# ethz-asl/ethzasl_brisk

Measured on AMD Instinct MI355X. Metric: frames/sec detect+describe @1080p (1/2/4/8 GPU); % HBM roofline, higher is better.
Workload: dtype u8

## Files before the change

ethzasl_brisk_amd/csrc/brisk_kernels.hip:

```cpp
#include <hip/hip_runtime.h>
#include <stdlib.h>

#include "brisk_common.h"
#include "brisk_device_detect.h"
#include "brisk_kernels.h"

#ifdef BRISK_HIP_TUNING
static int env_knob(const char* name, int dflt) {
  const char* v = getenv(name);
  return (v && *v) ? atoi(v) : dflt;
}
#else
#define env_knob(name, dflt) (dflt)
#endif


__device__ __forceinline__ BriskLayerView make_view(const BriskGeom& G, uint8_t* pyr, uint16_t* smap, int frame,
                                                    int l) {
  BriskLayerView v;
  const long base = (long)frame * G.pyr_elems + G.L[l].off;
  v.img = brisk_layer_img(G, pyr, frame, l);
  v.smap = smap + base;
  v.w = G.L[l].w;
  v.h = G.L[l].h;
// ... 940 lines not shown
      const int j = j0 + tid;
      const unsigned* t = tmp + ((long)l * n_in + j) * 8;
      const bool ok = j < cnt && t[7] != 0;
      const unsigned long long bal = __ballot(ok);
      if (lane == 0) wtot[wave] = __popcll(bal);
      __syncthreads();
      int wbase = 0, total = 0;
#pragma unroll
      for (int q = 0; q < 16; ++q) { wbase += (q < wave) ? wtot[q] : 0; total += wtot[q]; }
      const int pos = base + wbase + __popcll(bal & ((1ull << lane) - 1ull));
      if (ok && pos < kp_cap) {
        BriskKeyPoint kp;
        kp.x = __uint_as_float(t[0]); kp.y = __uint_as_float(t[1]); kp.size = __uint_as_float(t[2]); kp.angle = __uint_as_float(t[3]);
        kp.response = __uint_as_float(t[4]); kp.octave = (int)t[5]; kp.class_id = (int)t[6];
        kp_out[pos] = kp;
      }
      __syncthreads();
      if (tid == 0) base += total;
      __syncthreads();
    }
  }
  if (tid == 0) {
    counters[0].nkp = min(base, kp_cap);
    if (base > kp_cap) atomicOr(&counters[0].overflow, 4);
  }
}

__global__ void __launch_bounds__(64) k_compute_scale(BriskGeom G, uint8_t* pyr, uint16_t* smap, const BriskKeyPoint* in, int n_in,
                                                       int suppress, BriskFrameCounters* counters, unsigned* det_scratch,
                                                       int det_cap, BriskKeyPoint* kp_out, int kp_cap, int always) {
  if (threadIdx.x != 0 || blockIdx.x != 0) return;
  if (!always && !counters[0].pad[0]) return;
  counters[0].full_clear = 1;
  BriskOrderedOut out;
  out.kp = kp_out; out.cap = kp_cap; out.n = 0; out.mask = nullptr; out.mask_row_pitch = 0;
  bool cap_exceeded = false;
  const bool undefined = brisk_compute_scale_walk(G, pyr, smap, in, n_in, suppress != 0, det_scratch, det_cap, &out, &cap_exceeded);
  if (undefined) atomicOr(&counters[0].overflow, 16);
  if (cap_exceeded) atomicOr(&counters[0].overflow, 1);
  counters[0].nkp = min(out.n, kp_cap);
  if (out.n > kp_cap) atomicOr(&counters[0].overflow, 4);
}

#ifndef TR_WAVES
#define TR_WAVES 16
#endif
#define TR_THREADS (TR_WAVES * 64)
#define TR_WIN 9
#ifndef TR_CHUNK
#define TR_CHUNK 3072
#endif
#define TR_PROG_DONE 0x7FFFFFFF
#define TR_DONE_BIT 4
#define TR_BM_WORDS 512
#ifdef TR_TIMING
#define TR_T(i) { const long long now_ = (long long)wall_clock64(); tacc[i] += (int)(now_ - tlast); tlast = now_; }
#else
#define TR_T(i)
#endif
#ifdef TR_TIMELINE
#define TR_STAMP(c_, l_, k_) if (c_) counters[frame].tl[(l_) * 8 + (k_)] = (int)wall_clock64();
#else
#define TR_STAMP(c_, l_, k_)
#endif


#define TR_KERNEL_NAME k_tie_resolve
#define TR_SORT_NAME tie_sort_large
#define TR_KERNEL_MASKS 0
#define TR_KERNEL_PAIR 0
#include "brisk_tie_kernel.inc"
#undef TR_KERNEL_NAME
#undef TR_KERNEL_MASKS
#undef TR_SORT_NAME
#define TR_KERNEL_NAME k_tie_resolve_small
#define TR_SORT_NAME tie_sort_large_small
#define TR_KERNEL_MASKS 1
#include "brisk_tie_kernel.inc"
#undef TR_KERNEL_NAME
#undef TR_SORT_NAME
#undef TR_KERNEL_PAIR
#define TR_KERNEL_NAME k_tie_resolve_pair
#define TR_SORT_NAME tie_sort_large_pair
#define TR_KERNEL_PAIR 1
#include "brisk_tie_kernel.inc"
#undef TR_KERNEL_NAME
#undef TR_KERNEL_PAIR
#undef TR_KERNEL_MASKS

#ifndef FN_THREADS
#define FN_THREADS 512
#endif
#define FN_BUCKETS 2048
#define FN_SMALL 3072
#define FN_SB 1024
__global__ void __launch_bounds__(FN_THREADS) k_finalize(BriskGeom G, const BriskCand* cand, BriskFrameCounters* counters,
                                                          unsigned* keys_scratch, BriskKeyPoint* kp_out, int cand_cap,
                                                          int kp_cap, const uint8_t* mask, long mask_pitch_frame,
                                                          int mask_row_pitch) {
  __shared__ int nvalid;
  __shared__ unsigned skey[FN_SMALL];
  __shared__ unsigned sidx[FN_SMALL];
  BRISK_CHAIN_SETPRIO();
  const int frame = blockIdx.x, tid = threadIdx.x;
  if (counters[frame].low_score) return;
  const int n = min(counters[frame].ncand, cand_cap);
  const BriskCand* C = cand + (long)frame * cand_cap;
  unsigned* keys = keys_scratch + (long)frame * cand_cap * 2;
  if (tid == 0) nvalid = 0;
  __syncthreads();
  constexpr int FN_U = 4;
  for (int i0 = tid; i0 < n; i0 += FN_U * FN_THREADS) {
    unsigned sw[FN_U], ck[FN_U];
#pragma unroll
    for (int u = 0; u < FN_U; ++u) {
      const int i = min(i0 + u * FN_THREADS, n - 1);
      sw[u] = *reinterpret_cast<const unsigned*>(reinterpret_cast<const uint8_t*>(&C[i]) + 4);
      ck[u] = C[i].key;
    }
#pragma unroll
    for (int u = 0; u < FN_U; ++u) {
      const int i = i0 + u * FN_THREADS;
      bool valid = i < n && ((sw[u] >> 16) & 0xFFu) == BRISK_ST_PASS && ((sw[u] >> 24) & 1u);
      if (valid && mask) {
        const BriskCand& c = C[i];
        const uint8_t* m = mask + (long)frame * mask_pitch_frame;
        valid = m[(long)(int)(c.ky + 0.5f) * mask_row_pitch + (int)(c.kx + 0.5f)] != 0;
      }
      if (valid) {
        const int j = atomicAdd(&nvalid, 1);
        keys[2 * j] = ck[u];
        keys[2 * j + 1] = (unsigned)i;
        if (j < FN_SMALL) { skey[j] = ck[u]; sidx[j] = (unsigned)i; }
      }
    }
  }
  __threadfence_block();
  __syncthreads();
  const int nv = nvalid;
  if (nv > FN_SMALL) {
    if (tid == 0) counters[frame].nvalid_large = nv;
    return;
  }
  {
    __shared__ int rbase[BRISK_MAX_LAYERS + 1];
    __shared__ int bhead[FN_SB];
    __shared__ int bstart[FN_SB];
    __shared__ int bnext[FN_SMALL];
    __shared__ int wsum[FN_THREADS / 64];
    if (tid == 0) {
      int acc = 0;
      for (int l = 0; l < G.nlayers; ++l) { rbase[l] = acc; acc += G.L[l].h; }
      rbase[G.nlayers] = acc;
    }
    for (int b = tid; b < FN_SB; b += FN_THREADS) { bhead[b] = -1; bstart[b] = 0; }
    __syncthreads();
    int shift = 0;
    while ((rbase[G.nlayers] >> shift) >= FN_SB) ++shift;
    auto bucket_of = [&](unsigned key) { return (rbase[key >> 26] + (int)((key >> 13) & 0x1FFF)) >> shift; };
    for (int j = tid; j < nv; j += FN_THREADS) {
      const int b = bucket_of(skey[j]);
      atomicAdd(&bstart[b], 1);
      bnext[j] = atomicExch(&bhead[b], j);
    }
    __syncthreads();
    {
      constexpr int PER = FN_SB / FN_THREADS;
      int loc[PER], sum = 0;
#pragma unroll
      for (int q = 0; q < PER; ++q) { loc[q] = bstart[tid * PER + q]; sum += loc[q]; }
      const int incl = wave_inclusive_scan(sum);
      const int lane = tid & 63, wave = tid >> 6;
      if (lane == 63) wsum[wave] = incl;
      __syncthreads();
      int woff = 0;
#pragma unroll
      for (int q = 0; q < FN_THREADS / 64; ++q) woff += (q < wave) ? wsum[q] : 0;
      int run = woff + incl - sum;
#pragma unroll
      for (int q = 0; q < PER; ++q) { bstart[tid * PER + q] = run; run += loc[q]; }
    }
    __syncthreads();
    for (int j = tid; j < nv; j += FN_THREADS) {
      const unsigned k = skey[j];
      const BriskCand& c = C[sidx[j]];
      const float4 r = *reinterpret_cast<const float4*>(&c.kx);
      const int lyr = c.layer;
      const int b = bucket_of(k);
      int rank = bstart[b];
      for (int q = bhead[b]; q >= 0; q = bnext[q]) rank += (skey[q] < k) ? 1 : 0;
      if (rank < kp_cap) {
        BriskKeyPoint kp;
        kp.x = r.x; kp.y = r.y; kp.size = r.z; kp.angle = -1.0f; kp.response = r.w;
        kp.octave = G.single_layer ? 0 : lyr; kp.class_id = -1;
        kp_out[(long)frame * kp_cap + rank] = kp;
      }
    }
  }
  if (tid == 0) {
    counters[frame].nkp = min(nv, kp_cap);
    if (nv > kp_cap) atomicOr(&counters[frame].overflow, 4);
  }
}

__global__ void __launch_bounds__(FN_THREADS) k_finalize_large(BriskGeom G, const BriskCand* cand, BriskFrameCounters* counters,
                                                                const unsigned* keys_scratch, unsigned* scratch2,
                                                                long scratch2_stride, BriskKeyPoint* kp_out, int cand_cap,
                                                                int kp_cap) {
  const int frame = blockIdx.x, tid = threadIdx.x;
  const int nv = counters[frame].nvalid_large;
  if (nv <= 0) return;
  __shared__ int bstart[FN_BUCKETS + 1];
  __shared__ int bfill[FN_BUCKETS];
  __shared__ int rbase[BRISK_MAX_LAYERS + 1];
  __shared__ int wsum[FN_THREADS / 64];
  const BriskCand* C = cand + (long)frame * cand_cap;
  const unsigned* keys = keys_scratch + (long)frame * cand_cap * 2;
  unsigned* tmp = scratch2 + (long)frame * scratch2_stride;
  if (tid == 0) {
    int acc = 0;
    for (int l = 0; l < G.nlayers; ++l) { rbase[l] = acc; acc += G.L[l].h; }
    rbase[G.nlayers] = acc;
  }
  for (int b = tid; b < FN_BUCKETS; b += FN_THREADS) { bstart[b] = 0; bfill[b] = 0; }
  __syncthreads();
  int shift = 0;
  while ((rbase[G.nlayers] >> shift) >= FN_BUCKETS) ++shift;
  for (int j = tid; j < nv; j += FN_THREADS) {
    const unsigned key = keys[2 * j];
    atomicAdd(&bstart[(rbase[key >> 26] + (int)((key >> 13) & 0x1FFF)) >> shift], 1);
  }
  __syncthreads();
  {
    constexpr int PER = FN_BUCKETS / FN_THREADS;
    int loc[PER], sum = 0;
#pragma unroll
    for (int q = 0; q < PER; ++q) { loc[q] = bstart[tid * PER + q]; sum += loc[q]; }
    int incl = sum;
    const int lane = tid & 63, wave = tid >> 6;
#pragma unroll
    for (int off = 1; off < 64; off <<= 1) {
      const int v = __shfl_up(incl, off, 64);
      if (lane >= off) incl += v;
    }
    if (lane == 63) wsum[wave] = incl;
    __syncthreads();
    int woff = 0;
#pragma unroll
    for (int q = 0; q < FN_THREADS / 64; ++q) woff += (q < wave) ? wsum[q] : 0;
    int run = woff + incl - sum;
#pragma unroll
    for (int q = 0; q < PER; ++q) { bstart[tid * PER + q] = run; run += loc[q]; }
    if (tid == FN_THREADS - 1) bstart[FN_BUCKETS] = run;
  }
  __syncthreads();
  for (int j = tid; j < nv; j += FN_THREADS) {
    const unsigned key = keys[2 * j];
    const int b = (rbase[key >> 26] + (int)((key >> 13) & 0x1FFF)) >> shift;
    const int pos = bstart[b] + atomicAdd(&bfill[b], 1);
    tmp[2 * pos] = key;
    tmp[2 * pos + 1] = keys[2 * j + 1];
  }
  __threadfence();
  __syncthreads();
  for (int pos = tid; pos < nv; pos += FN_THREADS) {
    const unsigned key = tmp[2 * pos];
    const int b = (rbase[key >> 26] + (int)((key >> 13) & 0x1FFF)) >> shift;
    int rank = bstart[b];
    for (int q = bstart[b]; q < bstart[b + 1]; ++q) rank += (tmp[2 * q] < key) ? 1 : 0;
    if (rank < kp_cap) {
      const BriskCand& c = C[tmp[2 * pos + 1]];
      BriskKeyPoint kp;
      kp.x = c.kx; kp.y = c.ky; kp.size = c.ksize; kp.angle = -1.0f; kp.response = c.kresp;
      kp.octave = G.single_layer ? 0 : c.layer; kp.class_id = -1;
      kp_out[(long)frame * kp_cap + rank] = kp;
    }
  }
  if (tid == 0) {
    counters[frame].nkp = min(nv, kp_cap);
    if (nv > kp_cap) atomicOr(&counters[frame].overflow, 4);
  }
}

#define II_THREADS 512
#define II_BAND 64
#define II_CHUNK (II_THREADS * 4)

__device__ __forceinline__ unsigned ii_wg_scan(unsigned total, unsigned (*wave_tot)[II_THREADS / 64], int buf, unsigned* wg_total) {
  const int lane = threadIdx.x & 63, wave = threadIdx.x >> 6;
  const unsigned incl = (unsigned)wave_inclusive_scan((int)total);
  if (lane == 63) wave_tot[buf][wave] = incl;
  __syncthreads();
  unsigned woff = 0, tot = 0;
#pragma unroll
  for (int q = 0; q < II_THREADS / 64; ++q) {
    const unsigned v = wave_tot[buf][q];
    woff += (q < wave) ? v : 0;
    tot += v;
  }
  *wg_total = tot;
  return woff + incl - total;
}

#ifndef II_ROWS
#define II_ROWS 3
#endif
#define II_MAXCHUNKS 4
__device__ __forceinline__ uint2 ii_fetch(const uint8_t* row, int stride, int c0 ) {
  const int a = min(max(c0 - 4, 0), stride - 4), b = min(c0, stride - 4);
  return make_uint2(*reinterpret_cast<const unsigned*>(row + a), *reinterpret_cast<const unsigned*>(row + b));
}
__device__ __forceinline__ void ii_unpack(uint2 raw, int stride, int w, int c0, unsigned* px) {
  const unsigned prev = (c0 >= 4 && c0 - 4 < stride) ? raw.x : 0u, cur = (c0 < stride) ? raw.y : 0u;
  px[0] = (c0 - 1 >= 0 && c0 - 1 < w) ? (prev >> 24) : 0;
  px[1] = (c0 < w) ? (cur & 0xFF) : 0;
  px[2] = (c0 + 1 < w) ? ((cur >> 8) & 0xFF) : 0;
  px[3] = (c0 + 2 < w) ? ((cur >> 16) & 0xFF) : 0;
}

typedef uint32_t __attribute__((ext_vector_type(3))) ii_u32x3;
__device__ __forceinline__ void ii_store4(bool b24, uint32_t* out, long row, int istride, int c0, unsigned a0, unsigned a1, unsigned a2, unsigned a3) {
  if (b24) {
    ii_u32x3 v;
    v.x = (a0 & 0xFFFFFFu) | (a1 << 24);
    v.y = ((a1 >> 8) & 0xFFFFu) | (a2 << 16);
    v.z = ((a2 >> 16) & 0xFFu) | (a3 << 8);
    *reinterpret_cast<ii_u32x3*>(reinterpret_cast<uint8_t*>(out) + (row * istride + c0) * 3) = v;
  } else {
    *reinterpret_cast<uint4*>(out + row * istride + c0) = make_uint4(a0, a1, a2, a3);
  }
}
template <int NCH, bool B24, bool SUB>
__global__ void __launch_bounds__(II_THREADS) k_integral_final(BriskGeom G, const uint8_t* __restrict__ pyr,
                                                               const uint32_t* __restrict__ bandsum,
                                                               uint32_t* __restrict__ integral, int istride, long iframe_elems,
                                                               int nbands, int band_h, BriskFrameCounters* counters, int nsub, int sub_h) {
  __shared__ unsigned wave_tot[2][II_THREADS / 64];
  const int frame = blockIdx.y, band = SUB ? (int)blockIdx.x / nsub : (int)blockIdx.x;
  const int sub = SUB ? (int)blockIdx.x - band * nsub : 0;
  constexpr bool b24 = B24;
  if (counters && blockIdx.x == 0 && threadIdx.x == 0) counters[frame].i24 = b24 ? 1 : 0;
  const int w = G.L[0].w, h = G.L[0].h, stride = G.L[0].stride;
  const uint8_t* img = brisk_layer_img(G, pyr, frame, 0);
  uint32_t* out = integral + (long)frame * iframe_elems;
  const int yb = band * band_h;
  const int y0 = SUB ? yb + sub * sub_h : yb;
  const int y1 = SUB ? min(min(h, yb + band_h), y0 + sub_h) : min(h, y0 + band_h);
  if (SUB && y0 >= y1) return;
  int buf = 0;
  unsigned acc[NCH][4];
  uint2 raw[NCH];
#pragma unroll
  for (int ch = 0; ch < NCH; ++ch) raw[ch] = ii_fetch(img + (long)min(y0, h - 1) * stride, stride, ch * II_CHUNK + threadIdx.x * 4);
  {
    unsigned carry = 0;
#pragma unroll
    for (int ch = 0; ch < NCH; ++ch) {
      const int c0 = ch * II_CHUNK + threadIdx.x * 4;
      uint4 C = make_uint4(0, 0, 0, 0);
      if (c0 <= w)
        for (int b = 0; b < band; ++b) {
          const uint4 v = *reinterpret_cast<const uint4*>(bandsum + ((long)frame * nbands + b) * istride + c0);
          C.x += v.x; C.y += v.y; C.z += v.z; C.w += v.w;
        }
      if (SUB && c0 <= w) {
        for (int r0 = yb; r0 < y0; r0 += 6) {
          uint2 rr[6];
#pragma unroll
          for (int k = 0; k < 6; ++k) rr[k] = ii_fetch(img + (long)min(r0 + k, y0 - 1) * stride, stride, c0);
#pragma unroll
          for (int k = 0; k < 6; ++k) {
            unsigned px[4];
            ii_unpack(rr[k], stride, w, c0, px);
            if (r0 + k < y0) { C.x += px[0]; C.y += px[1]; C.z += px[2]; C.w += px[3]; }
          }
        }
      }
      if (c0 + 1 > w) C.y = 0;
      if (c0 + 2 > w) C.z = 0;
      if (c0 + 3 > w) C.w = 0;
      const unsigned s0 = C.x, s1 = s0 + C.y, s2 = s1 + C.z, s3 = s2 + C.w;
      unsigned tot;
      const unsigned o = ii_wg_scan(s3, wave_tot, buf, &tot) + carry;
      buf ^= 1;
      carry += tot;
      acc[ch][0] = o + s0; acc[ch][1] = o + s1; acc[ch][2] = o + s2; acc[ch][3] = o + s3;
      if (band == 0 && sub == 0 && c0 <= w) ii_store4(b24, out, 0, istride, c0, 0, 0, 0, 0);
    }
  }
  __shared__ unsigned wave_totr[2][II_THREADS / 64][II_ROWS];
  uint2 rawr[II_ROWS][NCH];
#pragma unroll
  for (int k = 0; k < II_ROWS; ++k)
#pragma unroll
    for (int ch = 0; ch < NCH; ++ch)
      rawr[k][ch] = (k == 0) ? raw[ch] : ii_fetch(img + (long)min(y0 + k, h - 1) * stride, stride, ch * II_CHUNK + threadIdx.x * 4);
  const int lane = threadIdx.x & 63, wave = threadIdx.x >> 6;
  for (int y = y0; y < y1; y += II_ROWS) {
    uint2 nxt[II_ROWS][NCH];
#pragma unroll
    for (int k = 0; k < II_ROWS; ++k) {
      const int yn = min(y + II_ROWS + k, y1 - 1);
#pragma unroll
      for (int ch = 0; ch < NCH; ++ch) nxt[k][ch] = ii_fetch(img + (long)yn * stride, stride, ch * II_CHUNK + threadIdx.x * 4);
    }
    unsigned carry[II_ROWS];
#pragma unroll
    for (int k = 0; k < II_ROWS; ++k) carry[k] = 0;
#pragma unroll
    for (int ch = 0; ch < NCH; ++ch) {
      const int c0 = ch * II_CHUNK + threadIdx.x * 4;
      unsigned s[II_ROWS][4], incl[II_ROWS];
#pragma unroll
      for (int k = 0; k < II_ROWS; ++k) {
        unsigned px[4] = {0, 0, 0, 0};
        if (c0 <= w && y + k < y1) ii_unpack(rawr[k][ch], stride, w, c0, px);
        s[k][0] = px[0]; s[k][1] = s[k][0] + px[1]; s[k][2] = s[k][1] + px[2]; s[k][3] = s[k][2] + px[3];
        incl[k] = (unsigned)wave_inclusive_scan((int)s[k][3]);
        if (lane == 63) wave_totr[buf][wave][k] = incl[k];
      }
      __syncthreads();
#pragma unroll
      for (int k = 0; k < II_ROWS; ++k) {
        unsigned wo = 0, tot = 0;
#pragma unroll
        for (int q = 0; q < II_THREADS / 64; ++q) {
          const unsigned v = wave_totr[buf][q][k];
          wo += (q < wave) ? v : 0;
          tot += v;
        }
        const unsigned o = wo + incl[k] - s[k][3] + carry[k];
        carry[k] += tot;
        acc[ch][0] += o + s[k][0]; acc[ch][1] += o + s[k][1]; acc[ch][2] += o + s[k][2]; acc[ch][3] += o + s[k][3];
        if (c0 <= w && y + k < y1) ii_store4(b24, out, (long)(y + k + 1), istride, c0, acc[ch][0], acc[ch][1], acc[ch][2], acc[ch][3]);
      }
      buf ^= 1;
    }
#pragma unroll
    for (int k = 0; k < II_ROWS; ++k)
#pragma unroll
      for (int ch = 0; ch < NCH; ++ch) rawr[k][ch] = nxt[k][ch];
  }
}

void brisk_launch_integral(const BriskGeom& G, const uint8_t* pyr, const uint32_t* bandsum, uint32_t* integral, int istride,
                            long iframe_elems, int band_h, int nframes, hipStream_t s, int ibits, BriskFrameCounters* counters) {
  const int nbands = (G.L[0].h + band_h - 1) / band_h;
  const int nchunks = (G.L[0].w + 1 + II_CHUNK - 1) / II_CHUNK;
  static const int sub_knob = env_knob("BRISK_II_SUB", -1);
  const int sub_h = ((sub_knob > 0 ? sub_knob : (band_h >= 96 ? 18 : 15)) + II_ROWS - 1) / II_ROWS * II_ROWS;
  const bool sub = sub_knob != 0 && nframes <= 4 && sub_h < band_h;
  const int nsub = sub ? (band_h + sub_h - 1) / sub_h : 1;
  const dim3 grid(nbands * nsub, nframes), block(II_THREADS);
  static const int pad_lds = env_knob("BRISK_II_LDS", 0);
  const bool b24 = ibits == 24 && counters;
#define II_LAUNCH1(NCH, LDS, B24_, SUB_)                                                                                                   \
  hipLaunchKernelGGL((k_integral_final<NCH, B24_, SUB_>), grid, block, LDS, s, G, pyr, bandsum, integral, istride, iframe_elems, nbands,   \
                     band_h, counters, nsub, sub_h);
#define II_LAUNCH(NCH, LDS)                                                                                                                  \
  if (b24) { if (sub) { II_LAUNCH1(NCH, LDS, true, true) } else { II_LAUNCH1(NCH, LDS, true, false) } }                                      \
  else { if (sub) { II_LAUNCH1(NCH, LDS, false, true) } else { II_LAUNCH1(NCH, LDS, false, false) } }
  if (nchunks <= 1) { II_LAUNCH(1, pad_lds) }
  else if (nchunks == 2) { II_LAUNCH(2, 0) }
  else { II_LAUNCH(II_MAXCHUNKS, 0) }
#undef II_LAUNCH
#undef II_LAUNCH1
}

__global__ void __launch_bounds__(256) k_batch_density(const BriskFrameCounters* __restrict__ counters, int nframes, int cand_cap,
                                                       long long* __restrict__ host_word) {
  __shared__ long long part[4];
  long long sum = 0;
  for (int f = threadIdx.x; f < nframes; f += 256) sum += min(counters[f].ncand, cand_cap);
  for (int off = 32; off > 0; off >>= 1) sum += __shfl_xor(sum, off, 64);
  if ((threadIdx.x & 63) == 0) part[threadIdx.x >> 6] = sum;
  __syncthreads();
  if (threadIdx.x == 0) {
    const long long total = part[0] + part[1] + part[2] + part[3];
    __hip_atomic_store(host_word, (total & 0xFFFFFFFFFFll) | ((long long)nframes << 40), __ATOMIC_RELAXED, __HIP_MEMORY_SCOPE_SYSTEM);
  }
}
void brisk_launch_batch_density(const BriskFrameCounters* counters, int nframes, int cand_cap, long long* host_word, hipStream_t s) {
  hipLaunchKernelGGL(k_batch_density, dim3(1), dim3(256), 0, s, counters, nframes, cand_cap, host_word);
}

__global__ void __launch_bounds__(256) k_publish_single(const BriskFrameCounters* __restrict__ counters, const BriskKeyPoint* __restrict__ kps,
                                                        const uint8_t* __restrict__ desc, int which, int max_kp, int dev_pitch,
                                                        uint8_t* host, unsigned o_cnt, unsigned o_kp, unsigned o_desc, int* done, unsigned seq) {
  const int tid = threadIdx.x, gt = blockIdx.x * blockDim.x + tid, gn = gridDim.x * blockDim.x;
  const int cnt = (counters[0].overflow & 7) ? 0 : (which ? counters[0].ndesc : counters[0].nkp);
  const bool fits = cnt <= max_kp;
  const int n = fits ? cnt : 0;
  if (blockIdx.x == 0)
    for (int i = tid; i < (int)(sizeof(BriskFrameCounters) / 4); i += blockDim.x)
      reinterpret_cast<int*>(host + o_cnt)[i] = reinterpret_cast<const int*>(counters)[i];
  {
    const int* src = reinterpret_cast<const int*>(kps);
    int* dst = reinterpret_cast<int*>(host + o_kp);
    const int nd = n * (int)(sizeof(BriskKeyPoint) / 4);
    for (int i = gt; i < nd; i += gn) dst[i] = src[i];
  }
  if (desc) {
    const uint2* src = reinterpret_cast<const uint2*>(desc);
    uint2* dst = reinterpret_cast<uint2*>(host + o_desc);
    const long nd = (long)n * dev_pitch / 8;
    for (long i = gt; i < nd; i += gn) dst[i] = src[i];
  }
  __threadfence_system();
  __syncthreads();
  if (tid == 0) {
    const int old = __hip_atomic_fetch_add(done, 1, __ATOMIC_ACQ_REL, __HIP_MEMORY_SCOPE_AGENT);
    if (old == (int)gridDim.x - 1) {
      __hip_atomic_store(done, 0, __ATOMIC_RELAXED, __HIP_MEMORY_SCOPE_AGENT);
      __threadfence_system();
      __hip_atomic_store(reinterpret_cast<unsigned*>(host), seq | (fits ? 0u : 0x80000000u), __ATOMIC_RELEASE, __HIP_MEMORY_SCOPE_SYSTEM);
    }
  }
}
void brisk_launch_publish_single(const BriskFrameCounters* counters, const BriskKeyPoint* kps, const uint8_t* desc, int which, int max_kp,
                                 int dev_pitch, int expect, uint8_t* host, unsigned o_cnt, unsigned o_kp, unsigned o_desc, int* done,
                                 unsigned seq, hipStream_t s) {
  const long bytes = (long)expect * ((long)sizeof(BriskKeyPoint) + (desc ? dev_pitch : 0));
  int grid = (int)((bytes + 16383) / 16384);
  grid = grid < 1 ? 1 : (grid > 32 ? 32 : grid);
  hipLaunchKernelGGL(k_publish_single, dim3(grid), dim3(256), 0, s, counters, kps, desc, which, max_kp, dev_pitch, host, o_cnt, o_kp, o_desc,
                     done, seq);
}

int brisk_device_cus() {
  static int cus[64] = {};
  int dev = 0;
  if (hipGetDevice(&dev) != hipSuccess || dev < 0 || dev >= 64) return 256;
  int v = __atomic_load_n(&cus[dev], __ATOMIC_RELAXED);
  if (!v) {
    hipDeviceProp_t prop;
    v = (hipGetDeviceProperties(&prop, dev) == hipSuccess && prop.multiProcessorCount > 0) ? prop.multiProcessorCount : 256;
    __atomic_store_n(&cus[dev], v, __ATOMIC_RELAXED);
  }
  return v;
}

static inline int grid_for(long items, int per_block, int cap) {
  long b = (items + per_block - 1) / per_block;
  if (b < 1) b = 1;
  if (b > cap) b = cap;
  return (int)b;
}

const char* brisk_stage_name(int i) {
  static const char* n[BRISK_PROF_STAGES] = {"k_pyramid", "k_detect", "k_classify_refine", "k_tie_resolve", "k_finalize",
                                             "k_postfilter", "k_integral_final", "k_desc_prepare", "k_describe"};
  return (i >= 0 && i < BRISK_PROF_STAGES) ? n[i] : "?";
}

void brisk_prof_begin_call(BriskProfiler* P) {
  if (!P || !P->on) return;
  if (!P->created) {
    for (int c = 0; c < BRISK_PROF_MAX_CALLS; ++c)
      for (int k = 0; k <= BRISK_PROF_STAGES; ++k) (void)hipEventCreate(&P->ev[c][k]);
    for (int c = 0; c < BRISK_PROF_MAX_CALLS; ++c)
      for (int k = 0; k < 2; ++k) (void)hipEventCreate(&P->side_ev[c][k]);
    P->created = true;
  }
  const int c = P->calls % BRISK_PROF_MAX_CALLS;
  for (int k = 0; k <= BRISK_PROF_STAGES; ++k) P->used[c][k] = false;
  P->side_used[c] = false;
}

void brisk_prof_mark_side(BriskProfiler* P, int which, hipStream_t side) {
  if (!P || !P->on) return;
  const int c = P->calls % BRISK_PROF_MAX_CALLS;
  (void)hipEventRecord(P->side_ev[c][which], side);
  if (which == 1) P->side_used[c] = true;
}

void brisk_prof_destroy(BriskProfiler* P) {
  if (!P || !P->created) return;
  for (int c = 0; c < BRISK_PROF_MAX_CALLS; ++c) {
    for (int k = 0; k <= BRISK_PROF_STAGES; ++k) (void)hipEventDestroy(P->ev[c][k]);
    for (int k = 0; k < 2; ++k) (void)hipEventDestroy(P->side_ev[c][k]);
  }
  P->created = false;
}

void brisk_prof_mark(BriskProfiler* P, int slot, hipStream_t s) {
  if (!P || !P->on) return;
  const int c = P->calls % BRISK_PROF_MAX_CALLS;
  (void)hipEventRecord(P->ev[c][slot], s);
  P->used[c][slot] = true;
}

__global__ void __launch_bounds__(256) k_stream_copy(const float4* __restrict__ in, float4* __restrict__ out, long n) {
  for (long i = (long)blockIdx.x * blockDim.x + threadIdx.x; i < n; i += (long)gridDim.x * blockDim.x) out[i] = in[i];
}
__global__ void __launch_bounds__(256) k_stream_read(const float4* __restrict__ in, float* __restrict__ out, long n) {
  float s = 0;
  for (long i = (long)blockIdx.x * blockDim.x + threadIdx.x; i < n; i += (long)gridDim.x * blockDim.x) {
    const float4 v = in[i];
    s += v.x + v.y + v.z + v.w;
  }
  if (s == 1.2345f) out[0] = s;
}
void brisk_launch_stream_probe(const void* a, void* b, size_t bytes, int mode, hipStream_t s) {
  const long n = (long)(bytes / 16);
  if (mode == 0) hipLaunchKernelGGL(k_stream_copy, dim3(4096), dim3(256), 0, s, (const float4*)a, (float4*)b, n);
  else hipLaunchKernelGGL(k_stream_read, dim3(4096), dim3(256), 0, s, (const float4*)a, (float*)b, n);
}

void brisk_launch_smap_clear(const BriskGeom& Gprev, const BriskDetectBuffers& B, int nframes, hipStream_t s) {
  if (nframes > 0) hipLaunchKernelGGL(k_smap_clear, dim3(16, nframes), dim3(256), 0, s, Gprev, B.smap, B.cand, B.counters, B.cand_cap);
}

static void launch_pyramid(const BriskGeom& G, const BriskDetectBuffers& B, int nframes, const uint8_t* frames, long frame_pitch,
                           int row_pitch, hipStream_t s) {
  {
    const int even_levels = G.nlayers >= 7 ? 3 : G.nlayers >= 5 ? 2 : G.nlayers >= 3 ? 1 : 0;
    const int odd_levels = G.nlayers >= 8 ? 3 : G.nlayers >= 6 ? 2 : G.nlayers >= 4 ? 1 : G.nlayers >= 2 ? 0 : -1;
    const int ftx = (G.L[0].stride + 95) / 96, fty = (G.L[0].h + PF_BAND - 1) / PF_BAND;
    hipLaunchKernelGGL(k_pyramid_fused, dim3(ftx * fty, nframes), dim3(256), 0, s, G, frames, frame_pitch, row_pitch, B.pyr,
                       even_levels, odd_levels, ftx, fty, B.bandsum, B.istride);
    for (int l = 8; l < G.nlayers; ++l) {
      const long items = (long)(G.L[l].stride / 4) * G.L[l].h;
      hipLaunchKernelGGL(k_pyramid_level, dim3(grid_for(items, 256, 2048), nframes), dim3(256), 0, s, G, B.pyr, l - 2, l, 0);
    }
  }
}

void brisk_launch_detect(const BriskGeom& G, const BriskTileTable& T, const BriskDetectBuffers& B, int nframes,
                         const uint8_t* frames, long frame_pitch, int row_pitch, const uint8_t* mask,
                         long mask_frame_pitch, int mask_row_pitch, hipStream_t s, BriskProfiler* prof,
                         const BriskOverlap* ov) {
  (void)hipMemsetAsync(B.counters, 0, sizeof(BriskFrameCounters) * (size_t)nframes, s);
  brisk_prof_mark(prof, BRISK_STG_PYRAMID, s);
  const int probe_stop = env_knob("BRISK_DETECT_PROBE", 0);
  if (probe_stop != 2) launch_pyramid(G, B, nframes, frames, frame_pitch, row_pitch, s);
  static const int fork_at = env_knob("BRISK_INTEGRAL_FORK", 0);
  auto fork_integral = [&]() {
    (void)hipEventRecord(ov->fork, s);
    (void)hipStreamWaitEvent(ov->side, ov->fork, 0);
    brisk_prof_mark_side(prof, 0, ov->side);
    brisk_launch_integral(G, B.pyr, B.bandsum, ov->Dd->integral, ov->Dd->istride, ov->Dd->iframe_elems, B.band_h, nframes, ov->side,
                          ov->Dd->ibits, B.counters);
    brisk_prof_mark_side(prof, 1, ov->side);
    (void)hipEventRecord(ov->join, ov->side);
  };
  if (ov && fork_at == 1) fork_integral();
  brisk_prof_mark(prof, BRISK_STG_DETECT, s);
  hipLaunchKernelGGL(k_detect, dim3((T.total_tiles + 7) / 8 * 8, nframes), dim3(256), 0, s, G, T, B.pyr, B.smap, B.cand, B.counters,
                     B.cand_cap);
  if (probe_stop) return;
  if (ov && fork_at == 2) fork_integral();
  brisk_prof_mark(prof, BRISK_STG_CLASSIFY, s);
  const bool ordered_all = G.no_scale_nms || G.lower_threshold != BRISK_LOWER_THRESHOLD;
  const bool ordered_some = !ordered_all && G.threshold < BRISK_FAST_PATH_MIN_THRESHOLD;
  auto launch_ordered = [&](int only_flagged) {
    const long row_stride = (long)BRISK_MAX_LAYERS * B.tie_cap;
    hipLaunchKernelGGL(k_order_candidates, dim3(nframes), dim3(OC_THREADS), 0, s, G, B.cand, B.counters, B.keys, B.tie_idx,
                       row_stride, B.cand_cap, only_flagged);
    hipLaunchKernelGGL(k_ordered_keypoints, dim3(nframes), dim3(64), 0, s, G, B.pyr, B.smap, B.cand, B.counters, B.keys, B.kp_out,
                       B.cand_cap, B.kp_cap, mask, mask_frame_pitch, mask_row_pitch, G.no_scale_nms, only_flagged);
  };
  if (ordered_all) {
    brisk_prof_mark(prof, BRISK_STG_TIES, s);
    if (ov && fork_at != 1 && fork_at != 2) fork_integral();
    launch_ordered(0);
    brisk_prof_mark(prof, BRISK_STG_FINALIZE, s);
    brisk_prof_mark(prof, BRISK_STG_POSTFILTER, s);
    return;
  }
  static const int sb_knob = env_knob("BRISK_SB_BLOCKS", 0), cr_knob = env_knob("BRISK_CR_BLOCKS", 0);
  const int sb_blocks = sb_knob ? sb_knob : (nframes > 64 ? (nframes >= 256 ? 32 : 64) : 256), cr_blocks = cr_knob ? cr_knob : (nframes >= 64 ? 24 : 64);
  {
    const int sb_bpf = grid_for(B.cand_cap, SB_WAVES * SB_PER_WAVE, sb_blocks), cr_bpf = grid_for(B.cand_cap, 64, cr_blocks);
    hipLaunchKernelGGL(k_score_blocks, dim3(xcd_grid(nframes, sb_bpf)), dim3(SB_WAVES * 64), 0, s, G, B.pyr, B.smap, B.cand,
                       B.counters, B.blocks, B.cand_cap, nframes, sb_bpf);
    hipLaunchKernelGGL(k_classify_refine, dim3(xcd_grid(nframes, cr_bpf)), dim3(64), 0, s, G, B.pyr, B.smap, B.cand, B.counters,
                       B.blocks, B.tie_idx, B.cand_cap, B.tie_cap, nframes, cr_bpf);
  }
  hipLaunchKernelGGL(k_classify_refine_direct, dim3(8, nframes), dim3(64), 0, s, G, B.pyr, B.smap, B.cand, B.counters,
                     B.tie_idx, B.cand_cap, B.tie_cap);
  brisk_prof_mark(prof, BRISK_STG_TIES, s);
  if (ov && fork_at == 0) fork_integral();
  {
    static const int lpw_knob = env_knob("BRISK_TR_LPW", 0);
    const int per_wg = G.nlayers > 8 ? 192 : 256;
    int lpw_auto = G.nlayers;
    for (int c = 1; c <= G.nlayers; ++c)
      if (nframes * ((G.nlayers + c - 1) / c) <= per_wg) { lpw_auto = c; break; }
    const int lpw = lpw_knob ? min(lpw_knob, G.nlayers) : (nframes * G.nlayers <= 512 ? 1 : lpw_auto);
    int tr_grid = (nframes >= 8 ? (nframes + 7) / 8 * 8 : nframes) * ((G.nlayers + lpw - 1) / lpw);
    static const int persist_knob = env_knob("BRISK_TR_PERSIST", -1), pgrid_env = env_knob("BRISK_TR_PGRID", 0);
    const int pgrid_knob = pgrid_env > 0 ? pgrid_env : brisk_device_cus();
    const int persist = persist_knob >= 0 ? persist_knob : (tr_grid > pgrid_knob ? 1 : 0);
    if (persist && tr_grid > pgrid_knob) tr_grid = pgrid_knob;
    static const int waves_knob = env_knob("BRISK_TR_WAVES", 0);
    const int tr_waves = waves_knob ? min(max(waves_knob, 2), TR_WAVES) : ((!persist && lpw >= G.nlayers && nframes >= 192) ? 12 : TR_WAVES);
    static const int pair_knob = env_knob("BRISK_TR_PAIR", 1);
    static const int pair_min_knob = env_knob("BRISK_TR_PAIR_MIN", 0);
    static const int pair_mode_knob = env_knob("BRISK_TR_PAIR_MODE", 1);
    const int pair_min = (pair_min_knob ? pair_min_knob : 4 * (tr_waves - 1)) | (pair_mode_knob << 16);
    static const int bands_knob = env_knob("BRISK_TR_BANDS", 0);
    int bands = 1;
    if (lpw == 1 && !persist) {
      bands = bands_knob ? min(max(bands_knob, 1), BRISK_TIE_MAX_BANDS) : (tr_grid * 8 <= pgrid_knob ? 8 : tr_grid * 4 <= pgrid_knob ? 4 : tr_grid * 2 <= pgrid_knob ? 2 : 1);
      if (tr_grid * bands > pgrid_knob) bands = 1;
    }
    if ((nframes <= 64 && pair_knob) || pair_knob == 2)
      hipLaunchKernelGGL(k_tie_resolve_pair, dim3(tr_grid * bands), dim3(tr_waves * 64), 0, s, G, B.pyr, B.smap, B.cand, B.counters, B.tie_idx,
                         B.blocks, B.keys, B.cand_cap, B.tie_cap, nframes, lpw, persist, pair_min, bands);
    else if (nframes < 32)
      hipLaunchKernelGGL(k_tie_resolve_small, dim3(tr_grid), dim3(tr_waves * 64), 0, s, G, B.pyr, B.smap, B.cand, B.counters, B.tie_idx,
                         B.blocks, B.keys, B.cand_cap, B.tie_cap, nframes, lpw, persist, 0, 1);
    else
      hipLaunchKernelGGL(k_tie_resolve, dim3(tr_grid), dim3(tr_waves * 64), 0, s, G, B.pyr, B.smap, B.cand, B.counters, B.tie_idx,
                         B.blocks, B.keys, B.cand_cap, B.tie_cap, nframes, lpw, persist, 0, 1);
  }
  brisk_prof_mark(prof, BRISK_STG_FINALIZE, s);
  hipLaunchKernelGGL(k_finalize, dim3(nframes), dim3(FN_THREADS), 0, s, G, B.cand, B.counters, B.keys, B.kp_out, B.cand_cap,
                     B.kp_cap, mask, mask_frame_pitch, mask_row_pitch);
  hipLaunchKernelGGL(k_finalize_large, dim3(nframes), dim3(FN_THREADS), 0, s, G, B.cand, B.counters, B.keys,
                     reinterpret_cast<unsigned*>(B.tie_idx), (long)BRISK_MAX_LAYERS * B.tie_cap, B.kp_out, B.cand_cap, B.kp_cap);
  if (ordered_some) launch_ordered(1);
  brisk_prof_mark(prof, BRISK_STG_POSTFILTER, s);
}

void brisk_launch_compute_scale(const BriskGeom& G, const BriskDetectBuffers& B, const uint8_t* frame, int row_pitch,
                                const BriskKeyPoint* d_in, int n_in, int suppress, hipStream_t s) {
  (void)hipMemsetAsync(B.counters, 0, sizeof(BriskFrameCounters), s);
  launch_pyramid(G, B, 1, frame, 0, row_pitch, s);
  static const int seq_knob = env_knob("BRISK_CS_SEQUENTIAL", 0);
  const bool parallel = !seq_knob && (long)G.nlayers * n_in <= 2L * B.cand_cap;
  if (parallel) {
    int* adm = reinterpret_cast<int*>(B.keys);
    unsigned* tmp = reinterpret_cast<unsigned*>(B.blocks);
    hipLaunchKernelGGL(k_cs_admit, dim3(G.nlayers), dim3(CS_THREADS), 0, s, G, B.pyr, B.smap, d_in, n_in, B.counters, adm);
    hipLaunchKernelGGL(k_cs_scores, dim3((n_in + CS_THREADS - 1) / CS_THREADS, G.nlayers), dim3(CS_THREADS), 0, s, G, B.pyr, B.smap, d_in,
                       n_in, B.counters, adm);
    hipLaunchKernelGGL(k_cs_refine, dim3((n_in + 63) / 64, G.nlayers), dim3(64), 0, s, G, B.pyr, B.smap, d_in, n_in, suppress, B.counters,
                       adm, tmp);
    hipLaunchKernelGGL(k_cs_emit, dim3(1), dim3(1024), 0, s, G, B.counters, tmp, n_in, B.kp_out, B.kp_cap);
  }
  hipLaunchKernelGGL(k_compute_scale, dim3(1), dim3(64), 0, s, G, B.pyr, B.smap, d_in, n_in, suppress, B.counters, B.keys,
                     2 * B.cand_cap, B.kp_out, B.kp_cap, parallel ? 0 : 1);
}

void brisk_launch_layer0_only(const BriskGeom& G, const BriskDetectBuffers& B, int nframes, const uint8_t* frames,
                              long frame_pitch, int row_pitch, hipStream_t s) {
  const int etx = (G.L[0].stride + 63) / 64, ety = (G.L[0].h + 63) / 64;
  hipLaunchKernelGGL(k_pyramid_even, dim3(etx * ety, nframes), dim3(256), 0, s, G, frames, frame_pitch, row_pitch, B.pyr, 0,
                     etx, ety, B.bandsum, B.istride);
}
```

Measured before the change: 79210.

## Restructure integral image row loop into row groups with packed segment scans

Replaces the 3-row software-pipelined integral image loop with groups of II_KEEP/NCH rows. Each thread loads its pixels once with alignbit and a precomputed mask. Per-wave row totals are computed with SAD and pair-packed 16-bit inclusive scans, and the cross-wave offsets are resolved by one small prefix pass per group. The goal is fewer __syncthreads, fewer wave scans and less address arithmetic. In exchange it raises register pressure, adds occupancy launch bounds for the single-chunk case, and changes the sub-band height default to 16.

```diff
diff --git a/ethzasl_brisk_amd/csrc/brisk_kernels.hip b/ethzasl_brisk_amd/csrc/brisk_kernels.hip
--- a/ethzasl_brisk_amd/csrc/brisk_kernels.hip
+++ b/ethzasl_brisk_amd/csrc/brisk_kernels.hip
@@ -1266,8 +1266,8 @@
   return woff + incl - total;
 }
 
-#ifndef II_ROWS
-#define II_ROWS 3
+#ifndef II_KEEP
+#define II_KEEP 16
 #endif
 #define II_MAXCHUNKS 4
 __device__ __forceinline__ uint2 ii_fetch(const uint8_t* row, int stride, int c0 ) {
@@ -1295,7 +1295,7 @@
   }
 }
 template <int NCH, bool B24, bool SUB>
-__global__ void __launch_bounds__(II_THREADS) k_integral_final(BriskGeom G, const uint8_t* __restrict__ pyr,
+__global__ void __launch_bounds__(II_THREADS, NCH == 1 ? 8 : 1) k_integral_final(BriskGeom G, const uint8_t* __restrict__ pyr,
                                                                const uint32_t* __restrict__ bandsum,
                                                                uint32_t* __restrict__ integral, int istride, long iframe_elems,
                                                                int nbands, int band_h, BriskFrameCounters* counters, int nsub, int sub_h) {
@@ -1313,9 +1313,6 @@
   if (SUB && y0 >= y1) return;
   int buf = 0;
   unsigned acc[NCH][4];
-  uint2 raw[NCH];
-#pragma unroll
-  for (int ch = 0; ch < NCH; ++ch) raw[ch] = ii_fetch(img + (long)min(y0, h - 1) * stride, stride, ch * II_CHUNK + threadIdx.x * 4);
   {
     unsigned carry = 0;
 #pragma unroll
@@ -1352,58 +1349,90 @@
       if (band == 0 && sub == 0 && c0 <= w) ii_store4(b24, out, 0, istride, c0, 0, 0, 0, 0);
     }
   }
-  __shared__ unsigned wave_totr[2][II_THREADS / 64][II_ROWS];
-  uint2 rawr[II_ROWS][NCH];
-#pragma unroll
-  for (int k = 0; k < II_ROWS; ++k)
-#pragma unroll
-    for (int ch = 0; ch < NCH; ++ch)
-      rawr[k][ch] = (k == 0) ? raw[ch] : ii_fetch(img + (long)min(y0 + k, h - 1) * stride, stride, ch * II_CHUNK + threadIdx.x * 4);
+  constexpr int GR = II_KEEP / NCH, NSEG = NCH * (II_THREADS / 64);
+  constexpr int BR = NCH == 1 ? 4 : 2, BR1 = NCH == 1 ? GR : 2;
+  static_assert(GR % BR == 0 && GR % BR1 == 0 && BR1 % 2 == 0, "rows are reduced in pairs");
+  __shared__ unsigned seg_tot[2][GR][NSEG];
   const int lane = threadIdx.x & 63, wave = threadIdx.x >> 6;
-  for (int y = y0; y < y1; y += II_ROWS) {
-    uint2 nxt[II_ROWS][NCH];
-#pragma unroll
-    for (int k = 0; k < II_ROWS; ++k) {
-      const int yn = min(y + II_ROWS + k, y1 - 1);
-#pragma unroll
-      for (int ch = 0; ch < NCH; ++ch) nxt[k][ch] = ii_fetch(img + (long)yn * stride, stride, ch * II_CHUNK + threadIdx.x * 4);
-    }
-    unsigned carry[II_ROWS];
-#pragma unroll
-    for (int k = 0; k < II_ROWS; ++k) carry[k] = 0;
-#pragma unroll
-    for (int ch = 0; ch < NCH; ++ch) {
-      const int c0 = ch * II_CHUNK + threadIdx.x * 4;
-      unsigned s[II_ROWS][4], incl[II_ROWS];
-#pragma unroll
-      for (int k = 0; k < II_ROWS; ++k) {
-        unsigned px[4] = {0, 0, 0, 0};
-        if (c0 <= w && y + k < y1) ii_unpack(rawr[k][ch], stride, w, c0, px);
-        s[k][0] = px[0]; s[k][1] = s[k][0] + px[1]; s[k][2] = s[k][1] + px[2]; s[k][3] = s[k][2] + px[3];
-        incl[k] = (unsigned)wave_inclusive_scan((int)s[k][3]);
-        if (lane == 63) wave_totr[buf][wave][k] = incl[k];
+  unsigned pmask[NCH], offa[NCH], offb[NCH], offo[NCH];
+#pragma unroll
+  for (int ch = 0; ch < NCH; ++ch) {
+    const int c0 = ch * II_CHUNK + threadIdx.x * 4;
+    offa[ch] = (unsigned)min(max(c0 - 4, 0), stride - 4);
+    offb[ch] = (unsigned)min(c0, stride - 4);
+    offo[ch] = (unsigned)c0 * (b24 ? 3u : 4u);
+    pmask[ch] = ((c0 >= 1 && c0 - 1 < w) ? 0xFFu : 0u) | ((c0 < w) ? 0xFF00u : 0u) | ((c0 + 1 < w) ? 0xFF0000u : 0u) | ((c0 + 2 < w) ? 0xFF000000u : 0u);
+  }
+  int gbuf = 0;
+  const int ys = __builtin_amdgcn_readfirstlane(y0), ye = __builtin_amdgcn_readfirstlane(y1);
+  const uint8_t* grow = img + (long)ys * stride;
+  uint8_t* gout = reinterpret_cast<uint8_t*>(out) + (long)(ys + 1) * istride * (b24 ? 3 : 4);
+  for (int y = ys; y < ye; y += GR, gbuf ^= 1, grow += (long)GR * stride, gout += (long)GR * istride * (b24 ? 3 : 4)) {
+    unsigned P[GR][NCH];
+#pragma unroll
+    for (int k0 = 0; k0 < GR; k0 += BR1) {
+#pragma unroll
+      for (int k = k0; k < k0 + BR1; ++k) {
+        const uint8_t* row = grow + (unsigned)(min(k, ye - 1 - y) * stride);
+#pragma unroll
+        for (int ch = 0; ch < NCH; ++ch) {
+          const int c0 = ch * II_CHUNK + threadIdx.x * 4;
+          (void)c0;
+          const unsigned lo = *reinterpret_cast<const unsigned*>(row + offa[ch]), hi = *reinterpret_cast<const unsigned*>(row + offb[ch]);
+          P[k][ch] = __builtin_amdgcn_alignbit(hi, lo, 24) & ((y + k < ye) ? pmask[ch] : 0u);
+        }
       }
-      __syncthreads();
-#pragma unroll
-      for (int k = 0; k < II_ROWS; ++k) {
-        unsigned wo = 0, tot = 0;
-#pragma unroll
-        for (int q = 0; q < II_THREADS / 64; ++q) {
-          const unsigned v = wave_totr[buf][q][k];
-          wo += (q < wave) ? v : 0;
-          tot += v;
+#pragma unroll
+      for (int k = k0; k < k0 + BR1; k += 2)
+#pragma unroll
+        for (int ch = 0; ch < NCH; ++ch) {
+          const unsigned two = __builtin_amdgcn_sad_u8(P[k][ch], 0u, 0u) | (__builtin_amdgcn_sad_u8(P[k + 1][ch], 0u, 0u) << 16);
+          const unsigned tot = (unsigned)wave_inclusive_scan((int)two);
+          if (lane == 63) { seg_tot[gbuf][k][ch * (II_THREADS / 64) + wave] = tot & 0xFFFFu; seg_tot[gbuf][k + 1][ch * (II_THREADS / 64) + wave] = tot >> 16; }
         }
-        const unsigned o = wo + incl[k] - s[k][3] + carry[k];
-        carry[k] += tot;
-        acc[ch][0] += o + s[k][0]; acc[ch][1] += o + s[k][1]; acc[ch][2] += o + s[k][2]; acc[ch][3] += o + s[k][3];
-        if (c0 <= w && y + k < y1) ii_store4(b24, out, (long)(y + k + 1), istride, c0, acc[ch][0], acc[ch][1], acc[ch][2], acc[ch][3]);
-      }
-      buf ^= 1;
-    }
-#pragma unroll
-    for (int k = 0; k < II_ROWS; ++k)
-#pragma unroll
-      for (int ch = 0; ch < NCH; ++ch) rawr[k][ch] = nxt[k][ch];
+      __builtin_amdgcn_sched_barrier(0);
+    }
+    __syncthreads();
+    if (threadIdx.x < GR) {
+      unsigned v[NSEG], run = 0;
+#pragma unroll
+      for (int q = 0; q < NSEG; ++q) v[q] = seg_tot[gbuf][threadIdx.x][q];
+#pragma unroll
+      for (int q = 0; q < NSEG; ++q) { seg_tot[gbuf][threadIdx.x][q] = run; run += v[q]; }
+    }
+    __syncthreads();
+#pragma unroll
+    for (int k0 = 0; k0 < GR; k0 += BR) {
+      unsigned left[BR][NCH];
+#pragma unroll
+      for (int k = 0; k < BR; ++k)
+#pragma unroll
+        for (int ch = 0; ch < NCH; ++ch) left[k][ch] = seg_tot[gbuf][k0 + k][ch * (II_THREADS / 64) + wave];
+#pragma unroll
+      for (int k = k0; k < k0 + BR; ++k)
+#pragma unroll
+        for (int ch = 0; ch < NCH; ++ch) {
+          const int c0 = ch * II_CHUNK + threadIdx.x * 4;
+          const unsigned p = P[k][ch];
+          const unsigned s0 = p & 0xFFu, s1 = s0 + ((p >> 8) & 0xFFu), s2 = s1 + ((p >> 16) & 0xFFu), s3 = s2 + (p >> 24);
+          const unsigned o = left[k - k0][ch] + (unsigned)wave_inclusive_scan((int)s3) - s3;
+          acc[ch][0] += o + s0; acc[ch][1] += o + s1; acc[ch][2] += o + s2; acc[ch][3] += o + s3;
+          if (c0 <= w && y + k < ye) {
+            uint8_t* orow = gout + (unsigned)(k * istride * (b24 ? 3 : 4));
+            const unsigned a0 = acc[ch][0], a1 = acc[ch][1], a2 = acc[ch][2], a3 = acc[ch][3];
+            if (b24) {
+              ii_u32x3 v;
+              v.x = (a0 & 0xFFFFFFu) | (a1 << 24);
+              v.y = ((a1 >> 8) & 0xFFFFu) | (a2 << 16);
+              v.z = ((a2 >> 16) & 0xFFu) | (a3 << 8);
+              *reinterpret_cast<ii_u32x3*>(orow + offo[ch]) = v;
+            } else {
+              *reinterpret_cast<uint4*>(orow + offo[ch]) = make_uint4(a0, a1, a2, a3);
+            }
+          }
+        }
+      __builtin_amdgcn_sched_barrier(0);
+    }
   }
 }
 
@@ -1411,9 +1440,10 @@
                             long iframe_elems, int band_h, int nframes, hipStream_t s, int ibits, BriskFrameCounters* counters) {
   const int nbands = (G.L[0].h + band_h - 1) / band_h;
   const int nchunks = (G.L[0].w + 1 + II_CHUNK - 1) / II_CHUNK;
-  static const int sub_knob = env_knob("BRISK_II_SUB", -1);
-  const int sub_h = ((sub_knob > 0 ? sub_knob : (band_h >= 96 ? 18 : 15)) + II_ROWS - 1) / II_ROWS * II_ROWS;
-  const bool sub = sub_knob != 0 && nframes <= 4 && sub_h < band_h;
+  static const int sub_knob = env_knob("BRISK_II_SUB", -1), sub_frames_knob = env_knob("BRISK_II_SUB_FRAMES", 4);
+  const int group_rows = II_KEEP / (nchunks <= 1 ? 1 : nchunks == 2 ? 2 : II_MAXCHUNKS);
+  const int sub_h = ((sub_knob > 0 ? sub_knob : 16) + group_rows - 1) / group_rows * group_rows;
+  const bool sub = sub_knob != 0 && nframes <= sub_frames_knob && sub_h < band_h;
   const int nsub = sub ? (band_h + sub_h - 1) / sub_h : 1;
   const dim3 grid(nbands * nsub, nframes), block(II_THREADS);
   static const int pad_lds = env_knob("BRISK_II_LDS", 0);
```

Measured after the change: 79870, median of 6. Within noise of the previous version (+0.8%).
